# PKU-Alignment/SafeVLA

Measured on AMD Instinct MI355X. Metric: env-steps/sec through PPO-Lagrangian update, higher is better.
Workload: dtype bf16

## Files before the change

include/svla.h:

```cpp
#ifndef SVLA_H
#define SVLA_H
#include <stdint.h>
#ifdef __cplusplus
extern "C" {
#endif

typedef uint16_t svla_bf16;

typedef struct svla_dropout { unsigned seed, stream; float p; int row_mult; const unsigned* seed_dev; } svla_dropout;

int svla_gae_scan_f32(const float* rewards, const float* costs, const float* values, const float* c_values,
                      const float* masks, const float* next_v, const float* next_cv, double gamma, double tau, int T, int B,
                      float* ret, float* adv, float* c_ret, float* c_adv, void* stream);

int svla_ppo_lag_loss_fwd_bwd_f32(const float* logits, const float* values, const int64_t* actions, const float* old_logp,
                                  const float* adv, const float* c_adv, const float* returns, const float* old_values,
                                  int rows, int A, float lam, float clip, float value_coef, float action_w, float ent_coef,
                                  int use_clipped_value, float inv_n, float* dlogits, float* dvalues, double* sums,
                                  void* stream);
int svla_value_mse_fwd_bwd_f32(const float* values, const float* returns, const float* old_values, float clip, int rows, float coef,
                               float inv_n, float* dvalues, double* sums, void* stream);
int svla_hlgauss_fwd_bwd_f32(const float* logits, const float* target, const float* dvalue, int rows, int NB, float vmin, float vmax,
                             float sigma, float coef, float inv_n, float* values_out, float* dlogits, double* sums, void* stream);
int svla_ce_loss_fwd_bwd_f32(const float* logits, const long* target, int rows, int A, long ignore_index, const float* n_valid,
                             float* dlogits, double* sums, void* stream);

int svla_small_linear_fwd_f32(const float* x, const float* W, const float* bias, int rows, int N, int D, int T, int B,
                              float* out, void* stream);
int svla_small_linear_bwd_f32(const float* x, const float* W, const float* dout, int rows, int N, int D, int T, int B,
                              int accumulate_dx, float* dx, float* dW, float* db, void* stream);

int svla_norm_fwd_bf16(const svla_bf16* x, int xG, int xGS, int xOFF, const float* gamma, const float* beta, float eps, int rows,
                       int D, int rms, int relu, const float* tok, int tok_group, svla_bf16* y, int yG, int yGS, int yOFF,
                       float* mean, float* rstd, void* stream);
int svla_norm_bwd_bf16(const svla_bf16* dy, int dyG, int dyGS, int dyOFF, const svla_bf16* x, int xG, int xGS, int xOFF,
                       const float* gamma, const float* beta, const float* mean, const float* rstd, int rows, int D, int rms,
                       int relu, int tok_group, const svla_bf16* dres, svla_bf16* dx, int dxG, int dxGS, int dxOFF, float* dgamma,
                       float* dbeta, float* dtok, svla_bf16* dx_drop, const svla_dropout* drop, void* stream);

#define SVLA_RELU_BITS_BYTES(M, N) ((((long)(M) + 31) / 32) * 32 * ((long)(N) / 8))
int svla_gemm_nt_bf16(const svla_bf16* A, long lda, const svla_bf16* B, long ldb, const float* bias, const svla_bf16* residual,
                      long ldr, const svla_bf16* relu_mask, long ldm, void* C, long ldc, int M, int N, int K, int act,
                      int out_f32, float alpha, unsigned char* relu_bits_out, const unsigned char* relu_bits,
                      const svla_dropout* drop, void* stream);
int svla_gemm_force_small_tile(int on);
int svla_gemm_nt_rmsa_bf16(const svla_bf16* A, long lda, const svla_bf16* B, long ldb, const float* bias, const svla_bf16* residual, long ldr,
                           void* C, long ldc, int M, int N, int K, int act, float eps, const svla_dropout* drop, void* stream);
int svla_gemm_last_kernel(char* name, int cap, int* mnk);
int svla_asm_launch_raw(const char* name, const void* kernarg, int kernarg_bytes, int grid, int block, void* stream);
int svla_gemm_tn_f32acc(const svla_bf16* dY, long ldy, const svla_bf16* X, long ldx, float* dW, long ldw, float* db, int M, int N,
                        int K, void* stream);
int svla_colsum_bf16(const svla_bf16* dY, long ldy, int M, int N, int row_stride, float* db, void* stream);

int svla_gemm_f32(const float* A, long sam, long sak, const float* B, long sbn, long sbk, const float* bias, const float* residual,
                  long ldr, const float* mask, long ldm, float* C, long ldc, int M, int N, int K, int act, int accumulate, float alpha,
                  const svla_dropout* drop, void* stream);
int svla_colsum_f32(const float* X, long ldx, int M, int N, int row_stride, float* out, void* stream);

int svla_attn_fwd_bf16(const svla_bf16* Q, const svla_bf16* K, const svla_bf16* V, long ld, svla_bf16* O, long ldo, float* LSE,
                       int rows, int S, int H, int head_dim, float scale, int mask_mode, const int* traj, const float* bias,
                       const unsigned char* kvalid, int Sq, long ldq, int kv_rows, const svla_dropout* drop, void* stream);
int svla_attn_bwd_bf16(const svla_bf16* Q, const svla_bf16* K, const svla_bf16* V, long ld, const svla_bf16* O, long ldo,
                       const float* LSE, const svla_bf16* dO, long lddo, svla_bf16* dQ, svla_bf16* dK, svla_bf16* dV, long ldd,
                       int rows, int S, int H, int head_dim, float scale, int mask_mode, const int* traj, const float* bias,
                       const unsigned char* kvalid, int Sq, long ldq, long lddq, float* D_ws, const svla_dropout* drop,
                       void* stream);
int svla_attn_bwd_two_pass(int on);

int svla_replay_calls(int n, const int* fn_ids, const int* arg_offsets, const unsigned long long* args, int* failed_at);

int svla_acting_stage(const void* tok_src, void* tok_dst, long tok_bytes, const int64_t* pa_src, int64_t* pa_dst, const float* mask_src, float* mask_dst,
                      const int64_t* hand_src, int64_t* hand_dst, const int64_t* ts_src, int64_t* ts_dst, const int64_t* ids_src, int64_t* ids_dst, int64_t* am_dst,
                      unsigned char* am8_dst, unsigned char* kvalid_dst, int64_t* t_dev, int B, int L, int max_steps, int t, int* seed0, int* seed1, int* seed2,
                      int seed_inc, void* stream);

int svla_group_begin(int members);
int svla_group_member(int member);
int svla_group_end(void* stream);
int svla_group_stats(long* grouped, long* single);
int svla_replay_calls_grouped(int n, int members, const int* fn_ids, const int* arg_offsets, const unsigned long long* const* args, void* stream,
                              int* failed_at);
int svla_replay_abi_stamp(unsigned long long* stamp);

int svla_det_config(int slot, float* f32_base, long long* i64_shadow, long n);
int svla_det_finalize(float* f32, long long* i64_shadow, long n, void* stream);
int svla_det_bypass_count(unsigned long long* count, int reset);
int svla_det_set_grid(int frac_bits);

int svla_attn_fp8_quant(const svla_bf16* qkv, long ld, int rows, int S, int H, int head_dim, unsigned char* ws, float* scales,
                        void* stream);
int svla_attn_fp8_fwd(const unsigned char* ws, const float* scales, svla_bf16* O, long ldo, float* LSE, int rows, int S, int H,
                      int head_dim, float scale, const svla_dropout* drop, void* stream);
int svla_attn_fp8_bwd(const unsigned char* ws, const float* scales, const svla_bf16* O, long ldo, const float* LSE, const svla_bf16* dO,
                      long lddo, unsigned char* gws, float* gscale, float* D, svla_bf16* dQ, svla_bf16* dK, svla_bf16* dV, long ldd,
                      int rows, int S, int H, int head_dim, float scale, const svla_dropout* drop, void* stream);

int svla_feat_to_tokens(const float* feat, int R, int C, int P, int cam, int ncam, svla_bf16* out, void* stream);
int svla_fusion_fill(const float* fusion_token, const svla_bf16* text, const int* gid, int R, int S, int L, int text_off, int D,
                     svla_bf16* x0, void* stream);
int svla_fusion_text_bwd(const svla_bf16* dx0, const int* gid, int T, int B, int S, int L, int text_off, int D, float* dtext,
                         void* stream);
int svla_decoder_embed_fwd(const svla_bf16* xf, long xf_row_stride, const float* act_tab, const float* hand_tab,
                           const float* div_term, const int64_t* prev_actions, const float* masks, const int64_t* hand,
                           const int64_t* time_step, int T, int B, int n_actions, int D, svla_bf16* out, void* stream);
int svla_decoder_embed_bwd(const svla_bf16* dout, const int64_t* prev_actions, const float* masks, const int64_t* hand, int T,
                           int B, int n_actions, int D, svla_bf16* dxf, long dxf_row_stride, float* d_act_tab, float* d_hand_tab,
                           void* stream);
int svla_rows_add_bf16(svla_bf16* dst, long dst_ld, const svla_bf16* src, long src_ld, int rows, int D, void* stream);
int svla_zero_bytes(void* p, long bytes, void* stream);
int svla_kv_append_bf16(const svla_bf16* src, long ld_src, svla_bf16* cache, long cache_rows, int width, const int64_t* t_dev, int B,
                        void* stream);
int svla_swiglu_fwd(const svla_bf16* ab, long M, int Hd, svla_bf16* g, void* stream);
int svla_swiglu_bwd(const svla_bf16* ab, const svla_bf16* dg, long M, int Hd, svla_bf16* dab, void* stream);
int svla_row_hash_u8(const unsigned char* rows, long n_rows, int row_bytes, int64_t* out, void* stream);
int svla_embed_gather_f32_bf16(const float* table, const int64_t* ids, long n, int D, svla_bf16* out, void* stream);

int svla_normalize_u8_f32(const unsigned char* x, long n, const float* mean3, const float* std3, float* y, void* stream);
int svla_patchify_u8_bf16(const unsigned char* frames, int B, int H, int W, int crop_x, int P, int gh, int gw, int KP,
                          const float* mean3, const float* std3, svla_bf16* out, void* stream);
int svla_vit_tokens(const svla_bf16* patch, const float* cls, const float* pos, int B, int NP, int C, svla_bf16* y, void* stream);
// ... 75 lines not shown
```

safevla_amd/model.py:

```python
import math
import os
from typing import Dict, List, Optional, Tuple

import numpy as np

import torch
import torch.nn as nn

from . import ops
from .api import CategoricalDistr, SafeActorCriticOutput
from .losses import HLGaussLoss
from .text import GoalTokenizer, bytes_to_str

N_ACTIONS = 20
D = 512
DINO = 384
NPATCH = 84
TEXT_OFF = 1 + 2 * NPATCH
MAX_ACTING_WINDOW = 1024
TEXT_ENCODER_DIMS = {"t5-small": 512, "SigLIPBase": 768, "SigLIPLarge": 1024}
BF16, F32 = torch.bfloat16, torch.float32
import os as _os0
_NO_COMPRESSOR_BITS = _os0.environ.get("SVLA_NO_COMPRESSOR_BITS", "0") == "1"

# ... 57 lines not shown
    if init == "ones":
        return torch.ones(shape)
    if init == "zeros":
        return torch.zeros(shape)
    if init == "tok":
        return 0.1 * torch.rand(shape, generator=g)
    if init == "emb":
        return (torch.rand(shape, generator=g) * 2 - 1) * 0.01
    if init == "lin":
        fan_in = int(np.prod(shape[1:]))
        return (torch.rand(shape, generator=g) * 2 - 1) / math.sqrt(fan_in)
    if init == "actor":
        w = torch.empty(shape)
        nn.init.orthogonal_(w, gain=0.01)
        return w
    if init == "critic":
        w = torch.empty(shape)
        nn.init.orthogonal_(w)
        return w
    raise KeyError(init)


class Tower(nn.Module):

    def __init__(self, arena: _Arena, device, n_fusion_layers=3, n_decoder_layers=3, max_steps=500, critic_type="linear",
                 precision="bf16", dino_dim=DINO, text_encoder="t5-small", d_model=512, n_heads=8, n_heads_decoder=None):
        super().__init__()
        n_heads_decoder = n_heads if n_heads_decoder is None else n_heads_decoder
        if d_model % 64 or d_model > 1024 or d_model % n_heads or d_model % n_heads_decoder or max(d_model // n_heads, d_model // n_heads_decoder) > 128:
            raise NotImplementedError(f"transformer width {d_model} with {n_heads} / {n_heads_decoder} heads")
        D = self.D = d_model
        H = self.H = n_heads
        self.Hdec = n_heads_decoder
        self.hdim, self.hdim_dec = d_model // n_heads, d_model // n_heads_decoder
        HD = self.dec_hidden = 256 * ((int(2 * 4 * d_model / 3) + 255) // 256)
        self.dino_dim = dino_dim
        if text_encoder not in TEXT_ENCODER_DIMS:
            raise NotImplementedError("Only SigLIP and T5 text encoders are supported.")
        self.text_encoder_name, self.text_dim = text_encoder, TEXT_ENCODER_DIMS[text_encoder]
        if precision not in ("bf16", "fp32"):
            raise ValueError(f"precision must be 'bf16' (MFMA product path) or 'fp32' (verification mode), got {precision!r}")
        self.precision, self.adt = precision, (F32 if precision == "fp32" else BF16)
        if critic_type not in ("linear", "mlp", "discrete"):
            print(f"Unknown critic type: {critic_type}")
            raise NotImplementedError
        self.critic_type = critic_type
        self.arena = arena
        self.device_ = device
        if not 1 <= int(max_steps) <= MAX_ACTING_WINDOW:
            raise ValueError(f"max_steps = {max_steps}: the KV-cache window of the acting step is limited to {MAX_ACTING_WINDOW} steps")
        self.max_steps = max_steps
        self.time_step_counter = 0
        self.prune_last = True
        self.fp8_attention = False
        self.dropout_p = 0.1
        self.t5_dropout = True
        self.drop_seed_base = 0x5AFE + 977 * len(arena.specs)
        self._fwd_count = 0
        dec = arena.declare
        ve = self.visual_encoder = _NS()
        dec(ve, "fusion_token", (D,), "tok")
        dec(ve, "visual_sensor_token_raw_navigation_camera", (D,), "tok")
        dec(ve, "visual_sensor_token_raw_manipulation_camera", (D,), "tok")
        ve.text_adapter = _seq(3)
        dec(ve.text_adapter[0], "weight", (D, self.text_dim), "lin"); dec(ve.text_adapter[0], "bias", (D,), "zeros")
        dec(ve.text_adapter[1], "weight", (D,), "ones"); dec(ve.text_adapter[1], "bias", (D,), "zeros")
        ve.visual_compressor = _seq(4)
        dec(ve.visual_compressor[0], "weight", (D, dino_dim, 1, 1), "lin"); dec(ve.visual_compressor[0], "bias", (D,), "zeros")
        dec(ve.visual_compressor[2], "weight", (D, D, 1, 1), "lin"); dec(ve.visual_compressor[2], "bias", (D,), "zeros")
        ve.visual_adapter = _seq(3)
        dec(ve.visual_adapter[0], "weight", (D, D), "lin"); dec(ve.visual_adapter[0], "bias", (D,), "zeros")
        dec(ve.visual_adapter[1], "weight", (D,), "ones"); dec(ve.visual_adapter[1], "bias", (D,), "zeros")
        ve.fusion_xformer = _NS()
        ve.fusion_xformer.layers = nn.ModuleList()
        for _ in range(n_fusion_layers):
            l = _NS()
            l.self_attn = _NS()
            dec(l.self_attn, "in_proj_weight", (3 * D, D), "lin"); dec(l.self_attn, "in_proj_bias", (3 * D,), "zeros")
            l.self_attn.out_proj = _NS()
            dec(l.self_attn.out_proj, "weight", (D, D), "lin"); dec(l.self_attn.out_proj, "bias", (D,), "zeros")
            l.linear1 = _NS(); dec(l.linear1, "weight", (2048, D), "lin"); dec(l.linear1, "bias", (2048,), "zeros")
            l.linear2 = _NS(); dec(l.linear2, "weight", (D, 2048), "lin"); dec(l.linear2, "bias", (D,), "zeros")
            l.norm1 = _NS(); dec(l.norm1, "weight", (D,), "ones"); dec(l.norm1, "bias", (D,), "zeros")
            l.norm2 = _NS(); dec(l.norm2, "weight", (D,), "ones"); dec(l.norm2, "bias", (D,), "zeros")
            ve.fusion_xformer.layers.append(l)
        if text_encoder == "t5-small":
            ve.text_encoder = T5Frozen(device)
        else:
            from .siglip_text import SIGLIP_TEXT_PRESETS, SigLIPTextFrozen
            ve.text_encoder = SigLIPTextFrozen(device, **SIGLIP_TEXT_PRESETS[text_encoder])
        self.object_in_hand_embed = _NS(); dec(self.object_in_hand_embed, "weight", (3, D), "emb")
        self.last_actions_embed = _NS(); dec(self.last_actions_embed, "weight", (N_ACTIONS + 2, D), "emb")
        self.time_encoder = _NS()
        self.time_encoder.register_buffer("div_term", torch.exp(torch.arange(0, D, 2) * (-math.log(10000.0) / D)).to(device))
        self.decoder = _NS()
        self.decoder.layers = nn.ModuleList()
        for _ in range(n_decoder_layers):
            l = _NS()
            l.attention = _NS()
            for n in ("wq", "wk", "wv"):
                setattr(l.attention, n, _NS()); dec(getattr(l.attention, n), "weight", (D, D), "lin")
            l.attention.wo = _NS(); dec(l.attention.wo, "weight", (D, D), "lin")
            l.feed_forward = _NS()
            l.feed_forward.w1 = _NS(); l.feed_forward.w2 = _NS(); l.feed_forward.w3 = _NS()
            dec(l.feed_forward.w1, "weight", (HD, D), "lin")
            dec(l.feed_forward.w3, "weight", (HD, D), "lin")
# ... 90 lines not shown

    def _ensure_caches(self, B: int):
        D, H, HD = self.D, self.H, self.dec_hidden
        if getattr(self, "_kv", None) is None or self._kv[0].shape[0] < B:
            self._kv_version = getattr(self, "_kv_version", 0) + 1
            self._kv = [torch.zeros(B, self.max_steps, 2 * D, device=self.device_, dtype=self.adt) for _ in self.decoder.layers]

    def cache_select(self, keep: list):
        if getattr(self, "_kv", None) is not None:
            idx = torch.as_tensor(keep, device=self.device_, dtype=torch.long)
            self._kv = [c[idx].contiguous() for c in self._kv]
            self._kv_version = getattr(self, "_kv_version", 0) + 1

    def run_forward(self, prep: "Prep", need_grad: bool):
        D, H, HD = self.D, self.H, self.dec_hidden
        SCF, SCD = self.hdim ** -0.5, self.hdim_dec ** -0.5
        T, B, R, S, L, U = prep.T, prep.B, prep.R, prep.S, prep.L, prep.U
        if T > 1 or need_grad or not getattr(prep, "acting", True) or self.time_step_counter >= self.max_steps:
            self.time_step_counter = 0
        ve, w = self.visual_encoder, self._w
        M2, M = R * 2 * NPATCH, R * S
        c = {}
        c["drop_seed"], site = self._drop_sites()
        tok = prep.tokens.view(M2, self.dino_dim)
        bits = need_grad and self.adt == BF16 and not _NO_COMPRESSOR_BITS
        c1b = torch.empty(ops.relu_bits_bytes(M2, D), device=self.device_, dtype=torch.uint8) if bits else None
        c2b = torch.empty(ops.relu_bits_bytes(M2, D), device=self.device_, dtype=torch.uint8) if bits else None
        c1 = ops.gemm_nt(tok, w["c1"], M2, D, self.dino_dim, bias=ve.visual_compressor[0].bias, act=ops.ACT_RELU, relu_bits_out=c1b)
        c2 = ops.gemm_nt(c1, w["c2"], M2, D, D, bias=ve.visual_compressor[2].bias, act=ops.ACT_RELU, relu_bits_out=c2b)
        a1 = ops.gemm_nt(c2, w["va"], M2, D, D, bias=ve.visual_adapter[0].bias)
        x = torch.empty(R, S, D, device=self.device_, dtype=self.adt)
        _, va_mean, va_rstd = ops.norm_fwd(a1, ve.visual_adapter[1].weight, ve.visual_adapter[1].bias, 1e-5, M2, relu=True,
                                           tok=self._camtok, tok_group=NPATCH, y=x, ymap=(2 * NPATCH, S, 1), D=D)
        t5_seed = c["drop_seed"] if self.t5_dropout else None
        key = getattr(prep, "ids_key", None)
        if t5_seed is None and key is not None and getattr(self, "_t5_cache", (None, None))[0] == key:
            t5 = self._t5_cache[1]
        else:
            t5 = ve.text_encoder.encode(prep.ids, getattr(prep, "attn_mask_u8", None) if getattr(prep, "attn_mask_u8", None) is not None else prep.attn_mask,
                                        drop_seed=t5_seed, drop_p=self.dropout_p, dtype=self.adt,
                                        seed_dev=getattr(self, "_seed_dev", None), fused=getattr(self, "t5_fused", None))
            self._t5_cache = (key, t5) if (t5_seed is None and key is not None) else (None, None)
        ta = ops.gemm_nt(t5, w["ta"], U * L, D, self.text_dim, bias=ve.text_adapter[0].bias)
        tf, ta_mean, ta_rstd = ops.norm_fwd(ta, ve.text_adapter[1].weight, ve.text_adapter[1].bias, 1e-5, U * L, relu=True, D=D)
        ops.fusion_fill(ve.fusion_token, tf, prep.gid, x, R, S, L, TEXT_OFF)
        c.update(c1=c1, c2=c2, c1b=c1b, c2b=c2b, a1=a1, va=(va_mean, va_rstd), t5=t5, ta=ta, ta_stats=(ta_mean, ta_rstd))
        xf = x.view(M, D)
        fl = []
        nfl = len(ve.fusion_xformer.layers)
        xf_stride = S * D
        for i, l in enumerate(ve.fusion_xformer.layers):
            if i == nfl - 1 and self.prune_last:
                b_in = l.self_attn.in_proj_bias
                kv = ops.gemm_nt(xf, w[f"f{i}.in"][D:], M, 2 * D, D, bias=b_in[D:])
                q0 = ops.gemm_nt(xf, w[f"f{i}.in"][:D], R, D, D, bias=b_in[:D], lda=S * D)
                ao, lse = ops.attn_fwd(q0, kv, kv[:, D:], 2 * D, R, S, H, SCF, save_lse=need_grad, Sq=1, ldq=D, drop=site(i, 0), head_dim=self.hdim)
                h1 = ops.gemm_nt(ao, w[f"f{i}.out"], R, D, D, bias=l.self_attn.out_proj.bias, residual=xf, ldr=S * D, drop=site(i, 1, S))
                x1, m1, r1 = ops.norm_fwd(h1, l.norm1.weight, l.norm1.bias, 1e-5, R, save_stats=need_grad, D=D)
                f1 = ops.gemm_nt(x1, w[f"f{i}.l1"], R, 2048, D, bias=l.linear1.bias, act=ops.ACT_RELU, drop=site(i, 2, S))
                h2 = ops.gemm_nt(f1, w[f"f{i}.l2"], R, D, 2048, bias=l.linear2.bias, residual=x1, drop=site(i, 3, S))
                xo, m2, r2 = ops.norm_fwd(h2, l.norm2.weight, l.norm2.bias, 1e-5, R, save_stats=need_grad, D=D)
                if need_grad:
                    fl.append(dict(pruned=True, x=xf, kv=kv, q0=q0, ao=ao, lse=lse, h1=h1, x1=x1, n1=(m1, r1), f1=f1, h2=h2, n2=(m2, r2)))
                xf, xf_stride = xo, D
                continue
            qkv = ops.gemm_nt(xf, w[f"f{i}.in"], M, 3 * D, D, bias=l.self_attn.in_proj_bias)
            f8 = None
            if self.fp8_attention and self.adt == BF16 and S <= 256 and self.hdim == 64:
                f8 = ops.attn_fp8_quant(qkv, 3 * D, R, S, H)
                ao, lse = ops.attn_fp8_fwd(f8, SCF, save_lse=need_grad, drop=site(i, 0))
                qkv = None
            else:
                ao, lse = ops.attn_fwd(qkv, qkv[:, D:], qkv[:, 2 * D:], 3 * D, R, S, H, SCF, save_lse=need_grad, drop=site(i, 0), head_dim=self.hdim)
            h1 = ops.gemm_nt(ao, w[f"f{i}.out"], M, D, D, bias=l.self_attn.out_proj.bias, residual=xf, drop=site(i, 1))
            x1, m1, r1 = ops.norm_fwd(h1, l.norm1.weight, l.norm1.bias, 1e-5, M, save_stats=need_grad, D=D)
            f1b = torch.empty(ops.relu_bits_bytes(M, 2048), device=x1.device, dtype=torch.uint8) if (need_grad and self.adt == BF16) else None
            f1 = ops.gemm_nt(x1, w[f"f{i}.l1"], M, 2048, D, bias=l.linear1.bias, act=ops.ACT_RELU, relu_bits_out=f1b, drop=site(i, 2))
            h2 = ops.gemm_nt(f1, w[f"f{i}.l2"], M, D, 2048, bias=l.linear2.bias, residual=x1, drop=site(i, 3))
            xo, m2, r2 = ops.norm_fwd(h2, l.norm2.weight, l.norm2.bias, 1e-5, M, save_stats=need_grad, D=D)
            if need_grad:
                fl.append(dict(pruned=False, x=xf, qkv=qkv, f8=f8, ao=ao, lse=lse, h1=h1, x1=x1, n1=(m1, r1), f1=f1, f1b=f1b, h2=h2, n2=(m2, r2)))
            xf = xo
        c["fusion"] = fl
        j = torch.empty(R, D, device=self.device_, dtype=self.adt)
        ops.decoder_embed_fwd(xf, xf_stride, self.last_actions_embed.weight, self.object_in_hand_embed.weight,
                              self.time_encoder.div_term, prep.prev_actions, prep.masks, prep.hand, prep.time_step, T, B, j)
        xd = j
        dl = []
        if T == 1 and not need_grad and getattr(prep, "acting", True):
            if self.hdim_dec != 64:
                raise NotImplementedError("KV-cached single steps need 64-wide decoder heads (MFMA / decode attention kernels)")
            t = self.time_step_counter
            self._ensure_caches(B)
            t_dev = getattr(self, "_t_dev", None)
            if t_dev is None:
                start = torch.clamp(t - prep.time_step, min=0)
                kvalid = (torch.arange(t + 1, device=self.device_)[None, :] >= start[:, None]).to(torch.uint8).contiguous()
                S_att = t + 1
            else:
                kvalid = getattr(prep, "kvalid_static", None)
                if kvalid is None:
                    ar = self._ar_steps
                    kvalid = ((ar[None, :] <= t_dev) & (ar[None, :] >= torch.clamp(t_dev - prep.time_step, min=0)[:, None])).to(torch.uint8).contiguous()
                S_att = self.max_steps
            fused = self.adt == BF16 and getattr(self, "rms_fused", True)
            if fused:
                self.refresh_folded()
            for i, l in enumerate(self.decoder.layers):
                if fused:
                    qkv = ops.gemm_nt_rmsa(xd, self._wg[f"d{i}.qkv"], B, 3 * D, D, 1e-5)
                else:
                    n1, _, _ = ops.norm_fwd(xd, l.attention_norm.weight, None, 1e-5, B, rms=True, save_stats=False, D=D)
                    qkv = ops.gemm_nt(n1, w[f"d{i}.qkv"], B, 3 * D, D)
                cache = self._kv[i]
                if t_dev is None:
                    cache[:B, t].copy_(qkv[:, D:])
# ... 104 lines not shown
        ops.gemm_tn_acc(dy, c["nf"], dw["dout"], R, D, D)
        dnf = ops.gemm_nt(dy, wt["dout"], R, D, D)
        dx = ops.norm_bwd(dnf, c["xd_last"], self.decoder.norm.weight, None, None, c["rf"], R, g(self.decoder.norm.weight), None, rms=True, D=D)
        for i in reversed(range(len(self.decoder.layers))):
            l, a = self.decoder.layers[i], c["dec"][i]
            ops.gemm_tn_acc(dx, a["g"], dw[f"d{i}.w2"], R, D, HD)
            dg = ops.gemm_nt(dx, wt[f"d{i}.w2"], R, HD, D)
            dab = ops.swiglu_bwd(a["ab"], dg, R, HD)
            ops.gemm_tn_acc(dab, a["n2"], dw[f"d{i}.w13"], R, 2 * HD, D)
            dn2 = ops.gemm_nt(dab, wt[f"d{i}.w13"], R, D, 2 * HD)
            dh = ops.norm_bwd(dn2, a["h"], l.ffn_norm.weight, None, None, a["r2"], R, g(l.ffn_norm.weight), None, rms=True, dres=dx, D=D)
            ops.gemm_tn_acc(dh, a["ao"], dw[f"d{i}.wo"], R, D, D)
            dao = ops.gemm_nt(dh, wt[f"d{i}.wo"], R, D, D)
            dqkv = torch.empty(R, 3 * D, device=dev, dtype=self.adt)
            q = a["qkv"]
            ops.attn_bwd(q, q[:, D:], q[:, 2 * D:], 3 * D, a["ao"], D, a["lse"], dao, D, dqkv, dqkv[:, D:], dqkv[:, 2 * D:], 3 * D,
                         B, T, self.Hdec, SCD, mask_mode=ops.MASK_BLOCK_CAUSAL, traj=prep.traj_bt, head_dim=self.hdim_dec)
            ops.gemm_tn_acc(dqkv, a["n1"], dw[f"d{i}.qkv"], R, 3 * D, D)
            dn1 = ops.gemm_nt(dqkv, wt[f"d{i}.qkv"], R, D, 3 * D)
            dx = ops.norm_bwd(dn1, a["x"], l.attention_norm.weight, None, None, a["r1"], R, g(l.attention_norm.weight), None, rms=True, dres=dh, D=D)
        pruned = bool(c["fusion"]) and c["fusion"][-1]["pruned"]
        if pruned:
            dxf = torch.empty(R, D, device=dev, dtype=self.adt)
            ops.decoder_embed_bwd(dx, prep.prev_actions, prep.masks, prep.hand, T, B, dxf, D, g(self.last_actions_embed.weight),
                                  g(self.object_in_hand_embed.weight))
            dyf = dxf
        else:
            dxf = ops.zeros(R, S, D, device=dev, dtype=self.adt)
            ops.decoder_embed_bwd(dx, prep.prev_actions, prep.masks, prep.hand, T, B, dxf, S * D, g(self.last_actions_embed.weight),
                                  g(self.object_in_hand_embed.weight))
            dyf = dxf.view(M, D)
        site = self._site_fn(c.get("drop_seed"))
        drop_scale = 1.0 / (1.0 - self.dropout_p) if c.get("drop_seed") is not None else 1.0
        def masked_like(t, on):
            return torch.empty_like(t) if on else None
        for i in reversed(range(len(ve.fusion_xformer.layers))):
            l, a = ve.fusion_xformer.layers[i], c["fusion"][i]
            if a["pruned"]:
                d3, d1 = site(i, 3, S), site(i, 1, S)
                df = masked_like(a["h2"], d3 is not None)
                dh2 = ops.norm_bwd(dyf, a["h2"], l.norm2.weight, l.norm2.bias, a["n2"][0], a["n2"][1], R, g(l.norm2.weight), g(l.norm2.bias),
                                   dx_drop=df, drop=d3, D=D)
                df = dh2 if df is None else df
                ops.gemm_tn_acc(df, a["f1"], dw[f"f{i}.l2"], R, D, 2048, db=g(l.linear2.bias))
                df1 = ops.gemm_nt(df, wt[f"f{i}.l2"], R, 2048, D, relu_mask=a["f1"], alpha=drop_scale)
                ops.gemm_tn_acc(df1, a["x1"], dw[f"f{i}.l1"], R, 2048, D, db=g(l.linear1.bias))
                dx1 = ops.gemm_nt(df1, wt[f"f{i}.l1"], R, D, 2048, residual=dh2)
                da = masked_like(a["h1"], d1 is not None)
                dh1 = ops.norm_bwd(dx1, a["h1"], l.norm1.weight, l.norm1.bias, a["n1"][0], a["n1"][1], R, g(l.norm1.weight), g(l.norm1.bias),
                                   dx_drop=da, drop=d1, D=D)
                da = dh1 if da is None else da
                ops.gemm_tn_acc(da, a["ao"], dw[f"f{i}.out"], R, D, D, db=g(l.self_attn.out_proj.bias))
                dao = ops.gemm_nt(da, wt[f"f{i}.out"], R, D, D)
                dq0 = torch.empty(R, D, device=dev, dtype=self.adt)
                dkv = torch.empty(M, 2 * D, device=dev, dtype=self.adt)
                kv = a["kv"]
                ops.attn_bwd(a["q0"], kv, kv[:, D:], 2 * D, a["ao"], D, a["lse"], dao, D, dq0, dkv, dkv[:, D:], 2 * D, R, S, H, SCF, head_dim=self.hdim,
                             Sq=1, ldq=D, lddq=D, drop=site(i, 0))
                gb = g(l.self_attn.in_proj_bias)
                ops.gemm_tn_acc(dkv, a["x"], dw[f"f{i}.in"][D:], M, 2 * D, D, db=gb[D:])
                ops.gemm_tn_acc(dq0, a["x"], dw[f"f{i}.in"][:D], R, D, D, ldx=S * D, db=gb[:D])
                dyf = ops.gemm_nt(dkv, wt[f"f{i}.in"][:, D:], M, D, 2 * D)
                t0 = ops.gemm_nt(dq0, wt[f"f{i}.in"][:, :D], R, D, D, residual=dh1)
                ops.rows_add(dyf, S * D, t0, D, R, D)
                c["fusion"][i] = None
                continue
            d3, d1 = site(i, 3), site(i, 1)
            df = masked_like(a["h2"], d3 is not None)
            dh2 = ops.norm_bwd(dyf, a["h2"], l.norm2.weight, l.norm2.bias, a["n2"][0], a["n2"][1], M, g(l.norm2.weight), g(l.norm2.bias),
                               dx_drop=df, drop=d3, D=D)
            df = dh2 if df is None else df
            ops.gemm_tn_acc(df, a["f1"], dw[f"f{i}.l2"], M, D, 2048, db=g(l.linear2.bias))
            if a["f1b"] is not None:
                df1 = ops.gemm_nt(df, wt[f"f{i}.l2"], M, 2048, D, relu_bits=a["f1b"], alpha=drop_scale)
            else:
                df1 = ops.gemm_nt(df, wt[f"f{i}.l2"], M, 2048, D, relu_mask=a["f1"], alpha=drop_scale)
            ops.gemm_tn_acc(df1, a["x1"], dw[f"f{i}.l1"], M, 2048, D, db=g(l.linear1.bias))
            dx1 = ops.gemm_nt(df1, wt[f"f{i}.l1"], M, D, 2048, residual=dh2)
            del df1, df
            da = masked_like(a["h1"], d1 is not None)
            dh1 = ops.norm_bwd(dx1, a["h1"], l.norm1.weight, l.norm1.bias, a["n1"][0], a["n1"][1], M, g(l.norm1.weight), g(l.norm1.bias),
                               dx_drop=da, drop=d1, D=D)
            da = dh1 if da is None else da
            ops.gemm_tn_acc(da, a["ao"], dw[f"f{i}.out"], M, D, D, db=g(l.self_attn.out_proj.bias))
            dao = ops.gemm_nt(da, wt[f"f{i}.out"], M, D, D)
            dqkv = torch.empty(M, 3 * D, device=dev, dtype=self.adt)
            q = a["qkv"]
            if a.get("f8") is not None:
                ops.attn_fp8_bwd(a["f8"], a["ao"], a["lse"], dao, dqkv, dqkv[:, D:], dqkv[:, 2 * D:], 3 * D, SCF, drop=site(i, 0))
            else:
                ops.attn_bwd(q, q[:, D:], q[:, 2 * D:], 3 * D, a["ao"], D, a["lse"], dao, D, dqkv, dqkv[:, D:], dqkv[:, 2 * D:], 3 * D,
                             R, S, H, SCF, drop=site(i, 0), head_dim=self.hdim)
            ops.gemm_tn_acc(dqkv, a["x"], dw[f"f{i}.in"], M, 3 * D, D, db=g(l.self_attn.in_proj_bias))
            dyf = ops.gemm_nt(dqkv, wt[f"f{i}.in"], M, D, 3 * D, residual=dh1)
            c["fusion"][i] = None
        dx0 = dyf
        ops.colsum_acc(dx0, g(ve.fusion_token), R, D, row_stride=S)
        dtf = ops.zeros(U * L, D, device=dev, dtype=F32)
        if ops.det_active():
            dtf_sh = torch.zeros(U * L * D, device=dev, dtype=torch.int64)
            ops.det_config(1, dtf, dtf_sh)
            try:
                ops.fusion_text_bwd(dx0, prep.gid, T, B, S, L, TEXT_OFF, dtf)
                ops.det_finalize(dtf, dtf_sh)
            finally:
                ops.det_config(1, None, None)
        else:
            ops.fusion_text_bwd(dx0, prep.gid, T, B, S, L, TEXT_OFF, dtf)
        dtf_b = torch.empty(U * L, D, device=dev, dtype=self.adt)
        ops.cast_bf16(dtf, dtf_b)
        dta = ops.norm_bwd(dtf_b, c["ta"], ve.text_adapter[1].weight, ve.text_adapter[1].bias, c["ta_stats"][0], c["ta_stats"][1], U * L,
                           g(ve.text_adapter[1].weight), g(ve.text_adapter[1].bias), relu=True, D=D)
        ops.gemm_tn_acc(dta, c["t5"], dw["ta"], U * L, D, self.text_dim, db=g(ve.text_adapter[0].bias))
        da1 = ops.norm_bwd(dx0, c["a1"], ve.visual_adapter[1].weight, ve.visual_adapter[1].bias, c["va"][0], c["va"][1], M2,
                           g(ve.visual_adapter[1].weight), g(ve.visual_adapter[1].bias), relu=True, dtok=self._dcamtok,
# ... 489 lines not shown
```

safevla_amd/ops.py:

```python
import ctypes
import os
import struct
from typing import Optional, Tuple

import torch

from ._lib import lib

BF16 = torch.bfloat16
F32 = torch.float32

MASK_NONE, MASK_BLOCK_CAUSAL = 0, 1
ACT_NONE, ACT_RELU, ACT_GELU = 0, 1, 2


class LaunchPlan:

    def __init__(self):
        self.calls, self.keep = [], []

    def __enter__(self):
        global _REC
        assert _REC is None and lib().recorder is None, "launch recording is not re-entrant"
        _REC = self
# ... 350 lines not shown
        return colsum_f32(dY, db, M, N, row_stride=row_stride, ldx=ldy if ldy is not None else dY.stride(-2))
    lib().call("svla_colsum_bf16", _p(dY), ldy if ldy is not None else dY.stride(-2), M, N, row_stride, _p(db), _stream())


def _f32_cols(t, W):
    return t[:, :W].float().contiguous()


def _attn96_on_mfma(S, bias) -> bool:
    return S <= 256 and bias is None and os.environ.get("SVLA_ATTN96_F32", "0") != "1"


def attn_fwd(q, k, v, ld, rows, S, H, scale, out=None, ldo=None, mask_mode=MASK_NONE, traj=None, bias=None, kvalid=None,
             save_lse=True, Sq=0, ldq=0, kv_rows=0, drop=None, head_dim=64):
    nq = Sq if Sq > 0 else S
    W = H * head_dim
    if head_dim != 64 and q.dtype != F32 and not (head_dim == 96 and _attn96_on_mfma(S, bias)):
        q32, k32, v32 = _f32_cols(q, W), _f32_cols(k, W), _f32_cols(v, W)
        o32, lse = attn_fwd(q32, k32, v32, W, rows, S, H, scale, mask_mode=mask_mode, traj=traj, bias=bias, kvalid=kvalid, save_lse=save_lse, Sq=Sq,
                            ldq=W if Sq > 0 else 0, kv_rows=kv_rows, drop=drop, head_dim=head_dim)
        if out is None:
            return o32.to(q.dtype), lse
        out[:, :W].copy_(o32)
        return out, lse
    if out is None:
        out = torch.empty(rows * nq, W, device=q.device, dtype=q.dtype)
    ldo = ldo if ldo is not None else out.stride(-2)
    lse = torch.empty(rows, H, nq, device=q.device, dtype=F32) if save_lse else None
    lib().call("svla_attn_fwd_f32" if q.dtype == F32 else "svla_attn_fwd_bf16", _p(q), _p(k), _p(v), ld, _p(out), ldo, _p(lse), rows, S, H, int(head_dim), float(scale), mask_mode,
               _p(traj), _p(bias), _p(kvalid), int(Sq), int(ldq), int(kv_rows), _d(drop), _stream())
    return out, lse


def attn_bwd(q, k, v, ld, o, ldo, lse, do, lddo, dq, dk, dv, ldd, rows, S, H, scale, mask_mode=MASK_NONE, traj=None,
             bias=None, kvalid=None, Sq=0, ldq=0, lddq=0, d_ws=None, drop=None, head_dim=64):
    if head_dim != 64 and q.dtype != F32 and not (head_dim == 96 and _attn96_on_mfma(S, bias)):
        W = H * head_dim
        q32, k32, v32, o32, do32 = (_f32_cols(t, W) for t in (q, k, v, o, do))
        dq32, dk32, dv32 = torch.empty_like(q32), torch.empty_like(k32), torch.empty_like(v32)
        attn_bwd(q32, k32, v32, W, o32, W, lse, do32, W, dq32, dk32, dv32, W, rows, S, H, scale, mask_mode=mask_mode, traj=traj, kvalid=kvalid, Sq=Sq,
                 ldq=W if Sq > 0 else 0, lddq=W if Sq > 0 else 0, drop=drop, head_dim=head_dim)
        dq[:, :W].copy_(dq32); dk[:, :W].copy_(dk32); dv[:, :W].copy_(dv32)
        return
    if q.dtype == F32:
        lib().call("svla_attn_bwd_f32", _p(q), _p(k), _p(v), ld, _p(o), ldo, _p(lse), _p(do), lddo, _p(dq), _p(dk), _p(dv), ldd, rows, S, H, int(head_dim),
                   float(scale), mask_mode, _p(traj), _p(kvalid), int(Sq), int(ldq), int(lddq), _d(drop), _stream())
        return
    if d_ws is None:
        d_ws = torch.empty(rows * H * (Sq or S), device=q.device, dtype=F32)
    lib().call("svla_attn_bwd_bf16", _p(q), _p(k), _p(v), ld, _p(o), ldo, _p(lse), _p(do), lddo, _p(dq), _p(dk), _p(dv), ldd,
               rows, S, H, int(head_dim), float(scale), mask_mode, _p(traj), _p(bias), _p(kvalid), int(Sq), int(ldq), int(lddq), _p(d_ws), _d(drop), _stream())


_DET_SLOTS = [None, None]


def det_config(slot: int, f32: Optional[torch.Tensor], shadow: Optional[torch.Tensor]) -> None:
    if f32 is None:
        lib().call("svla_det_config", int(slot), None, None, 0)
        _DET_SLOTS[slot] = None
        return
    assert f32.dtype == F32 and shadow.dtype == torch.int64 and shadow.numel() == f32.numel() and f32.is_contiguous()
    lib().call("svla_det_config", int(slot), f32.data_ptr(), shadow.data_ptr(), f32.numel())
    _DET_SLOTS[slot] = (f32, shadow)


def det_active() -> bool:
    return _DET_SLOTS[0] is not None


def det_finalize(f32: torch.Tensor, shadow: torch.Tensor) -> None:
    lib().call("svla_det_finalize", _p(f32), _p(shadow), f32.numel(), _stream())


def det_set_grid(frac_bits: int) -> None:
    lib().call("svla_det_set_grid", int(frac_bits))


def det_grid_bits(n_total: int) -> int:
    import math
    return max(36, min(52, 52 - max(0, math.ceil(math.log2(16384.0 / max(1, int(n_total)))))))


def det_bypass_count(reset: bool = True) -> int:
    c = ctypes.c_ulonglong(0)
    lib().call("svla_det_bypass_count", ctypes.byref(c), int(bool(reset)))
    return int(c.value)


def _fp8_sp(S: int) -> int:
    return 64 if S <= 64 else 128 if S <= 128 else 192 if S <= 192 else 256


class Fp8QKV:
    __slots__ = ("ws", "scales", "rows", "S", "H")

    def __init__(self, ws, scales, rows, S, H):
        self.ws, self.scales, self.rows, self.S, self.H = ws, scales, rows, S, H


def attn_fp8_quant(qkv, ld, rows, S, H) -> Fp8QKV:
    _chk(qkv, BF16, "qkv")
    ws = torch.empty(rows * H * 6 * _fp8_sp(S) * 64, device=qkv.device, dtype=torch.uint8)
    scales = torch.empty(rows * H * 3, device=qkv.device, dtype=F32)
    lib().call("svla_attn_fp8_quant", _p(qkv), ld, rows, S, H, 64, _p(ws), _p(scales), _stream())
    return Fp8QKV(ws, scales, rows, S, H)
# ... 311 lines not shown
```

Baseline: 7763.

## Absorb K/V projections into query for pruned last fusion layer attention

```diff
diff --git a/include/svla.h b/include/svla.h
--- a/include/svla.h
+++ b/include/svla.h
@@ -66,6 +66,12 @@
                        const unsigned char* kvalid, int Sq, long ldq, long lddq, float* D_ws, const svla_dropout* drop,
                        void* stream);
 int svla_attn_bwd_two_pass(int on);
+int svla_attn_q1_fwd_bf16(const svla_bf16* X, long ldx, const svla_bf16* QT, svla_bf16* C, float* SIG, float* P, int R, int S, float scale,
+                          const svla_dropout* drop, void* stream);
+int svla_attn_q1_bwd_bf16(const svla_bf16* X, long ldx, const svla_bf16* QT, const svla_bf16* DC, const float* DSIG, const float* P,
+                          svla_bf16* DX, long lddx, svla_bf16* DQT, int R, int S, float scale, const svla_dropout* drop, void* stream);
+int svla_head_expand_bf16(const svla_bf16* v, long ldv, int R, svla_bf16* E, const float* bias, float* dot, const float* sigma, svla_bf16* vs, void* stream);
+int svla_head_pick_bf16(const svla_bf16* G, int R, const float* sigma, const float* bias, svla_bf16* out, long ldo, void* stream);
 
 int svla_replay_calls(int n, const int* fn_ids, const int* arg_offsets, const unsigned long long* args, int* failed_at);
 
diff --git a/safevla_amd/csrc/attn_q1.hip b/safevla_amd/csrc/attn_q1.hip
--- /dev/null
+++ b/safevla_amd/csrc/attn_q1.hip
@@ -0,0 +1,303 @@
+#include "attn_common.h"
+
+#define Q1_D 512
+#define Q1_H 8
+#define Q1_WAVES 8
+#define Q1_THREADS (Q1_WAVES * 64)
+#define Q1_SMAX 256
+#define Q1_SLOTS (Q1_SMAX / Q1_WAVES)
+#define Q1_RED_FLOATS (Q1_H * Q1_D)
+#define Q1_LDS_FWD ((size_t)(Q1_SMAX * Q1_H + 4 * Q1_RED_FLOATS) * sizeof(float))
+#define Q1_LDS_BWD ((size_t)(2 * Q1_SMAX * Q1_H + 4 * Q1_RED_FLOATS) * sizeof(float))
+
+__device__ __forceinline__ void q1_unpack(bf16x8 v, float (&f)[8]) {
+    const u32x4 w = __builtin_bit_cast(u32x4, v);
+#pragma unroll
+    for (int i = 0; i < 4; ++i) { f[2 * i] = bf_lo(w[i]); f[2 * i + 1] = bf_hi(w[i]); }
+}
+
+__device__ __forceinline__ void q1_token_head_products(const bf16_t* __restrict__ X, const bf16_t* __restrict__ V, int S, float mul, float* out, int w, int lane) {
+    constexpr int NT = Q1_SMAX / (16 * Q1_WAVES), NK = Q1_D / 32;
+    const int ql = lane & 15, g = lane >> 4;
+    const bf16_t* vb = V + (size_t)(ql & (Q1_H - 1)) * Q1_D + 8 * g;
+    bf16x8 a[NT][NK], b[NK];
+#pragma unroll
+    for (int tt = 0; tt < NT; ++tt) {
+        const bf16_t* xa = X + (size_t)min((w + Q1_WAVES * tt) * 16 + ql, S - 1) * Q1_D + 8 * g;
+#pragma unroll
+        for (int kk = 0; kk < NK; ++kk) a[tt][kk] = *(const bf16x8*)(xa + kk * 32);
+    }
+#pragma unroll
+    for (int kk = 0; kk < NK; ++kk) b[kk] = *(const bf16x8*)(vb + kk * 32);
+#pragma unroll
+    for (int tt = 0; tt < NT; ++tt) {
+        const int j0 = (w + Q1_WAVES * tt) * 16;
+        f32x4 acc = {0.f, 0.f, 0.f, 0.f};
+#pragma unroll
+        for (int kk = 0; kk < NK; ++kk) acc = mfma16(a[tt][kk], b[kk], acc);
+        if (ql < Q1_H) {
+#pragma unroll
+            for (int i = 0; i < 4; ++i) {
+                const int j = j0 + 4 * g + i;
+                if (j < S) out[j * Q1_H + ql] = acc[i] * mul;
+            }
+        }
+    }
+}
+
+__device__ __forceinline__ void q1_load_slices(const bf16_t* __restrict__ X, int S, int w, int lane, bf16x8 (&xr)[Q1_SLOTS]) {
+#pragma unroll
+    for (int t = 0; t < Q1_SLOTS; ++t) {
+        const int j = min(w + Q1_WAVES * t, S - 1);
+        xr[t] = *(const bf16x8*)(X + (size_t)j * Q1_D + lane * 8);
+    }
+}
+
+__device__ __forceinline__ void q1_token_sums(const bf16x8 (&xr)[Q1_SLOTS], const float* coef, int S, int w, float (&acc)[Q1_H][8]) {
+#pragma unroll
+    for (int h = 0; h < Q1_H; ++h)
+#pragma unroll
+        for (int e = 0; e < 8; ++e) acc[h][e] = 0.f;
+#pragma unroll
+    for (int t = 0; t < Q1_SLOTS; ++t) {
+        const int j = w + Q1_WAVES * t;
+        if (j < S) {
+            const f32x4 c0 = *(const f32x4*)(coef + j * Q1_H), c1 = *(const f32x4*)(coef + j * Q1_H + 4);
+            float x[8];
+            q1_unpack(xr[t], x);
+#pragma unroll
+            for (int h = 0; h < 4; ++h)
+#pragma unroll
+                for (int e = 0; e < 8; ++e) { acc[h][e] += c0[h] * x[e]; acc[h + 4][e] += c1[h] * x[e]; }
+        }
+    }
+}
+
+__device__ __forceinline__ void q1_red_store(const float (&acc)[Q1_H][8], float* buf, int lane) {
+#pragma unroll
+    for (int h = 0; h < Q1_H; ++h) {
+        *(f32x4*)(buf + h * Q1_D + lane * 8) = f32x4{acc[h][0], acc[h][1], acc[h][2], acc[h][3]};
+        *(f32x4*)(buf + h * Q1_D + lane * 8 + 4) = f32x4{acc[h][4], acc[h][5], acc[h][6], acc[h][7]};
+    }
+}
+__device__ __forceinline__ void q1_red_add(float (&acc)[Q1_H][8], const float* buf, int lane) {
+#pragma unroll
+    for (int h = 0; h < Q1_H; ++h) {
+        const f32x4 a = *(const f32x4*)(buf + h * Q1_D + lane * 8), b = *(const f32x4*)(buf + h * Q1_D + lane * 8 + 4);
+#pragma unroll
+        for (int e = 0; e < 4; ++e) { acc[h][e] += a[e]; acc[h][e + 4] += b[e]; }
+    }
+}
+__device__ __forceinline__ void q1_reduce_write(float (&acc)[Q1_H][8], float* red, int w, int lane, bf16_t* __restrict__ out) {
+    if (w >= 4) q1_red_store(acc, red + (w - 4) * Q1_RED_FLOATS, lane);
+    __syncthreads();
+    if (w < 4) q1_red_add(acc, red + w * Q1_RED_FLOATS, lane);
+    if (w == 2 || w == 3) q1_red_store(acc, red + w * Q1_RED_FLOATS, lane);
+    __syncthreads();
+    if (w < 2) q1_red_add(acc, red + (w + 2) * Q1_RED_FLOATS, lane);
+    if (w == 1) q1_red_store(acc, red + Q1_RED_FLOATS, lane);
+    __syncthreads();
+    if (w == 0) {
+        q1_red_add(acc, red + Q1_RED_FLOATS, lane);
+#pragma unroll
+        for (int h = 0; h < Q1_H; ++h) *(bf16x8*)(out + h * Q1_D + lane * 8) = pack8(acc[h]);
+    }
+}
+
+struct Q1Args {
+    const bf16_t* X; long ldx;
+    const bf16_t* QT;
+    bf16_t* C; float* SIG; float* P;
+    const bf16_t* DC; const float* DSIG;
+    bf16_t* DX; long lddx; bf16_t* DQT;
+    int S; float scale; DropCfg drop;
+};
+
+__global__ void __launch_bounds__(Q1_THREADS, 1) attn_q1_fwd_kernel(Q1Args p) {
+    extern __shared__ __attribute__((aligned(16))) char smem[];
+    float* sc = (float*)smem;
+    float* red = sc + Q1_SMAX * Q1_H;
+    const int w = __builtin_amdgcn_readfirstlane(threadIdx.x >> 6), lane = threadIdx.x & 63, S = p.S;
+    const size_t r = blockIdx.x;
+    const DropCfg drop = drop_resolve(p.drop);
+    const bf16_t* X = p.X + r * p.ldx;
+    q1_token_head_products(X, p.QT + r * (Q1_H * Q1_D), S, p.scale, sc, w, lane);
+    bf16x8 xr[Q1_SLOTS];
+    q1_load_slices(X, S, w, lane, xr);
+    __syncthreads();
+    {
+        const int h = w;
+        float v[Q1_SMAX / 64], m = -INFINITY, sum = 0.f, sig = 0.f;
+#pragma unroll
+        for (int i = 0; i < Q1_SMAX / 64; ++i) {
+            const int j = lane + 64 * i;
+            v[i] = j < S ? sc[j * Q1_H + h] : -INFINITY;
+            m = fmaxf(m, v[i]);
+        }
+        m = wave_max(m);
+#pragma unroll
+        for (int i = 0; i < Q1_SMAX / 64; ++i) { v[i] = __expf(v[i] - m); sum += v[i]; }
+        const float inv = 1.f / wave_sum(sum);
+        const unsigned long long e0 = att_drop_row(S, Q1_H, (int)r, h, 0);
+#pragma unroll
+        for (int i = 0; i < Q1_SMAX / 64; ++i) {
+            const int j = lane + 64 * i;
+            if (j < S) {
+                const float pr = v[i] * inv;
+                const float pd = (!drop.thr || att_keep1(drop, e0 + j)) ? pr * drop.scale : 0.f;
+                p.P[(r * Q1_H + h) * S + j] = pr;
+                sc[j * Q1_H + h] = pd;
+                sig += pd;
+            }
+        }
+        sig = wave_sum(sig);
+        if (lane == 0) p.SIG[r * Q1_H + h] = sig;
+    }
+    __syncthreads();
+    float acc[Q1_H][8];
+    q1_token_sums(xr, sc, S, w, acc);
+    q1_reduce_write(acc, red, w, lane, p.C + r * (Q1_H * Q1_D));
+}
+
+__global__ void __launch_bounds__(Q1_THREADS, 1) attn_q1_bwd_kernel(Q1Args p) {
+    extern __shared__ __attribute__((aligned(16))) char smem[];
+    float* dsb = (float*)smem;
+    float* pdb = dsb + Q1_SMAX * Q1_H;
+    float* red = pdb + Q1_SMAX * Q1_H;
+    const int w = __builtin_amdgcn_readfirstlane(threadIdx.x >> 6), lane = threadIdx.x & 63, S = p.S;
+    const size_t r = blockIdx.x;
+    const DropCfg drop = drop_resolve(p.drop);
+    const bf16_t* X = p.X + r * p.ldx;
+    q1_token_head_products(X, p.DC + r * (Q1_H * Q1_D), S, 1.f, dsb, w, lane);
+    bf16x8 xr[Q1_SLOTS];
+    q1_load_slices(X, S, w, lane, xr);
+    __syncthreads();
+    {
+        const int h = w;
+        const float dsig = p.DSIG[r * Q1_H + h];
+        const unsigned long long e0 = att_drop_row(S, Q1_H, (int)r, h, 0);
+        float pr[Q1_SMAX / 64], dp[Q1_SMAX / 64], delta = 0.f;
+#pragma unroll
+        for (int i = 0; i < Q1_SMAX / 64; ++i) {
+            const int j = lane + 64 * i;
+            pr[i] = 0.f; dp[i] = 0.f;
+            if (j < S) {
+                pr[i] = p.P[(r * Q1_H + h) * S + j];
+                const bool keep = !drop.thr || att_keep1(drop, e0 + j);
+                dp[i] = keep ? (dsb[j * Q1_H + h] + dsig) * drop.scale : 0.f;
+                pdb[j * Q1_H + h] = keep ? pr[i] * drop.scale : 0.f;
+                delta += pr[i] * dp[i];
+            }
+        }
+        delta = wave_sum(delta);
+#pragma unroll
+        for (int i = 0; i < Q1_SMAX / 64; ++i) {
+            const int j = lane + 64 * i;
+            if (j < S) dsb[j * Q1_H + h] = p.scale * pr[i] * (dp[i] - delta);
+        }
+    }
+    __syncthreads();
+    {
+        float acc[Q1_H][8];
+        q1_token_sums(xr, dsb, S, w, acc);
+        q1_reduce_write(acc, red, w, lane, p.DQT + r * (Q1_H * Q1_D));
+    }
+    float qf[Q1_H][8], cf[Q1_H][8];
+    const bf16_t* QT = p.QT + r * (Q1_H * Q1_D) + lane * 8;
+    const bf16_t* DC = p.DC + r * (Q1_H * Q1_D) + lane * 8;
+#pragma unroll
+    for (int h = 0; h < Q1_H; ++h) {
+        q1_unpack(*(const bf16x8*)(QT + h * Q1_D), qf[h]);
+        q1_unpack(*(const bf16x8*)(DC + h * Q1_D), cf[h]);
+    }
+    bf16_t* DX = p.DX + r * p.lddx;
+#pragma unroll 1
+    for (int j = w; j < S; j += Q1_WAVES) {
+        const f32x4 s0 = *(const f32x4*)(dsb + j * Q1_H), s1 = *(const f32x4*)(dsb + j * Q1_H + 4);
+        const f32x4 d0 = *(const f32x4*)(pdb + j * Q1_H), d1 = *(const f32x4*)(pdb + j * Q1_H + 4);
+        float o[8];
+#pragma unroll
+        for (int e = 0; e < 8; ++e) o[e] = 0.f;
+#pragma unroll
+        for (int h = 0; h < 4; ++h)
+#pragma unroll
+            for (int e = 0; e < 8; ++e) {
+                o[e] += s0[h] * qf[h][e] + d0[h] * cf[h][e];
+                o[e] += s1[h] * qf[h + 4][e] + d1[h] * cf[h + 4][e];
+            }
+        *(bf16x8*)(DX + (size_t)j * Q1_D + lane * 8) = pack8(o);
+    }
+}
+
+static bool q1_shape_ok(int R, int S, long ldx) { return R > 0 && S > 0 && S <= Q1_SMAX && ldx >= (long)S * Q1_D && ldx % 8 == 0; }
+
+extern "C" int svla_attn_q1_fwd_bf16(const bf16_t* X, long ldx, const bf16_t* QT, bf16_t* C, float* SIG, float* P, int R, int S, float scale,
+                                     const svla_dropout* drop, void* stream) {
+    if (!X || !QT || !C || !SIG || !P || !q1_shape_ok(R, S, ldx)) return SVLA_EINVAL;
+    Q1Args p{};
+    p.X = X; p.ldx = ldx; p.QT = QT; p.C = C; p.SIG = SIG; p.P = P; p.S = S; p.scale = scale; p.drop = drop_cfg(drop);
+    return svla_launch<attn_q1_fwd_kernel>(dim3(R), dim3(Q1_THREADS), Q1_LDS_FWD, (hipStream_t)stream, p);
+}
+
+extern "C" int svla_attn_q1_bwd_bf16(const bf16_t* X, long ldx, const bf16_t* QT, const bf16_t* DC, const float* DSIG, const float* P,
+                                     bf16_t* DX, long lddx, bf16_t* DQT, int R, int S, float scale, const svla_dropout* drop, void* stream) {
+    if (!X || !QT || !DC || !DSIG || !P || !DX || !DQT || !q1_shape_ok(R, S, ldx) || !q1_shape_ok(R, S, lddx)) return SVLA_EINVAL;
+    Q1Args p{};
+    p.X = X; p.ldx = ldx; p.QT = QT; p.DC = DC; p.DSIG = DSIG; p.P = (float*)P; p.DX = DX; p.lddx = lddx; p.DQT = DQT;
+    p.S = S; p.scale = scale; p.drop = drop_cfg(drop);
+    return svla_launch<attn_q1_bwd_kernel>(dim3(R), dim3(Q1_THREADS), Q1_LDS_BWD, (hipStream_t)stream, p);
+}
+
+__global__ void __launch_bounds__(256) head_expand_kernel(const bf16_t* __restrict__ v, long ldv, int R, bf16_t* __restrict__ E, const float* __restrict__ bias,
+                                                          float* __restrict__ dot, const float* __restrict__ sigma, bf16_t* __restrict__ vs) {
+    const size_t r = (size_t)blockIdx.x * 4 + (threadIdx.x >> 6);
+    const int lane = threadIdx.x & 63, hl = lane >> 3;
+    if (r >= (size_t)R) return;
+    const bf16x8 x = *(const bf16x8*)(v + r * ldv + lane * 8);
+    const bf16x8 z = {0, 0, 0, 0, 0, 0, 0, 0};
+#pragma unroll
+    for (int h = 0; h < Q1_H; ++h) *(bf16x8*)(E + (r * Q1_H + h) * Q1_D + lane * 8) = h == hl ? x : z;
+    if (!bias && !sigma) return;
+    float f[8];
+    q1_unpack(x, f);
+    if (bias) {
+        float s = 0.f;
+#pragma unroll
+        for (int e = 0; e < 8; ++e) s += f[e] * bias[lane * 8 + e];
+        s += __shfl_xor(s, 1, 64); s += __shfl_xor(s, 2, 64); s += __shfl_xor(s, 4, 64);
+        if ((lane & 7) == 0) dot[r * Q1_H + hl] = s;
+    }
+    if (sigma) {
+        const float sg = sigma[r * Q1_H + hl];
+#pragma unroll
+        for (int e = 0; e < 8; ++e) f[e] *= sg;
+        *(bf16x8*)(vs + r * Q1_D + lane * 8) = pack8(f);
+    }
+}
+__global__ void __launch_bounds__(256) head_pick_kernel(const bf16_t* __restrict__ G, int R, const float* __restrict__ sigma, const float* __restrict__ bias,
+                                                        bf16_t* __restrict__ out, long ldo) {
+    const size_t r = (size_t)blockIdx.x * 4 + (threadIdx.x >> 6);
+    const int lane = threadIdx.x & 63, hl = lane >> 3;
+    if (r >= (size_t)R) return;
+    bf16x8 x = *(const bf16x8*)(G + (r * Q1_H + hl) * Q1_D + lane * 8);
+    if (sigma) {
+        float f[8];
+        q1_unpack(x, f);
+        const float sg = sigma[r * Q1_H + hl];
+#pragma unroll
+        for (int e = 0; e < 8; ++e) f[e] += sg * bias[lane * 8 + e];
+        x = pack8(f);
+    }
+    *(bf16x8*)(out + r * ldo + lane * 8) = x;
+}
+
+extern "C" int svla_head_expand_bf16(const bf16_t* v, long ldv, int R, bf16_t* E, const float* bias, float* dot, const float* sigma, bf16_t* vs, void* stream) {
+    if (!v || !E || R <= 0 || ldv < Q1_D || ldv % 8 || (bias && !dot) || (sigma && !vs)) return SVLA_EINVAL;
+    hipLaunchKernelGGL(head_expand_kernel, dim3((R + 3) / 4), dim3(256), 0, (hipStream_t)stream, v, ldv, R, E, bias, dot, sigma, vs);
+    return svla_launch_status();
+}
+extern "C" int svla_head_pick_bf16(const bf16_t* G, int R, const float* sigma, const float* bias, bf16_t* out, long ldo, void* stream) {
+    if (!G || !out || R <= 0 || ldo < Q1_D || ldo % 8 || (sigma && !bias)) return SVLA_EINVAL;
+    hipLaunchKernelGGL(head_pick_kernel, dim3((R + 3) / 4), dim3(256), 0, (hipStream_t)stream, G, R, sigma, bias, out, ldo);
+    return svla_launch_status();
+}
diff --git a/safevla_amd/model.py b/safevla_amd/model.py
--- a/safevla_amd/model.py
+++ b/safevla_amd/model.py
@@ -133,6 +133,7 @@
         self.max_steps = max_steps
         self.time_step_counter = 0
         self.prune_last = True
+        self.absorb_last = _os0.environ.get("SVLA_LAST_LAYER_KV", "0") != "1"
         self.fp8_attention = False
         self.dropout_p = 0.1
         self.t5_dropout = True
@@ -329,16 +330,25 @@
         for i, l in enumerate(ve.fusion_xformer.layers):
             if i == nfl - 1 and self.prune_last:
                 b_in = l.self_attn.in_proj_bias
-                kv = ops.gemm_nt(xf, w[f"f{i}.in"][D:], M, 2 * D, D, bias=b_in[D:])
                 q0 = ops.gemm_nt(xf, w[f"f{i}.in"][:D], R, D, D, bias=b_in[:D], lda=S * D)
-                ao, lse = ops.attn_fwd(q0, kv, kv[:, D:], 2 * D, R, S, H, SCF, save_lse=need_grad, Sq=1, ldq=D, drop=site(i, 0), head_dim=self.hdim)
+                absorbed = need_grad and self.absorb_last and self.adt == BF16 and self.hdim == 64 and H == 8 and S <= 256
+                if absorbed:
+                    eq, _, _ = ops.head_expand(q0, R)
+                    qt = ops.gemm_nt(eq, self._wt[f"f{i}.in"][:, D:2 * D], 8 * R, D, D)
+                    cc, sig, prob = ops.attn_q1_fwd(xf, S * D, qt, R, S, SCF, drop=site(i, 0))
+                    ao = ops.head_pick(ops.gemm_nt(cc, w[f"f{i}.in"][2 * D:], 8 * R, D, D), R, sigma=sig, bias=b_in[2 * D:])
+                    att = dict(absorbed=True, eq=eq, qt=qt, cc=cc, sig=sig, prob=prob)
+                else:
+                    kv = ops.gemm_nt(xf, w[f"f{i}.in"][D:], M, 2 * D, D, bias=b_in[D:])
+                    ao, lse = ops.attn_fwd(q0, kv, kv[:, D:], 2 * D, R, S, H, SCF, save_lse=need_grad, Sq=1, ldq=D, drop=site(i, 0), head_dim=self.hdim)
+                    att = dict(absorbed=False, kv=kv, lse=lse)
                 h1 = ops.gemm_nt(ao, w[f"f{i}.out"], R, D, D, bias=l.self_attn.out_proj.bias, residual=xf, ldr=S * D, drop=site(i, 1, S))
                 x1, m1, r1 = ops.norm_fwd(h1, l.norm1.weight, l.norm1.bias, 1e-5, R, save_stats=need_grad, D=D)
                 f1 = ops.gemm_nt(x1, w[f"f{i}.l1"], R, 2048, D, bias=l.linear1.bias, act=ops.ACT_RELU, drop=site(i, 2, S))
                 h2 = ops.gemm_nt(f1, w[f"f{i}.l2"], R, D, 2048, bias=l.linear2.bias, residual=x1, drop=site(i, 3, S))
                 xo, m2, r2 = ops.norm_fwd(h2, l.norm2.weight, l.norm2.bias, 1e-5, R, save_stats=need_grad, D=D)
                 if need_grad:
-                    fl.append(dict(pruned=True, x=xf, kv=kv, q0=q0, ao=ao, lse=lse, h1=h1, x1=x1, n1=(m1, r1), f1=f1, h2=h2, n2=(m2, r2)))
+                    fl.append(dict(pruned=True, x=xf, q0=q0, ao=ao, **att, h1=h1, x1=x1, n1=(m1, r1), f1=f1, h2=h2, n2=(m2, r2)))
                 xf, xf_stride = xo, D
                 continue
             qkv = ops.gemm_nt(xf, w[f"f{i}.in"], M, 3 * D, D, bias=l.self_attn.in_proj_bias)
@@ -549,15 +559,27 @@
                 da = dh1 if da is None else da
                 ops.gemm_tn_acc(da, a["ao"], dw[f"f{i}.out"], R, D, D, db=g(l.self_attn.out_proj.bias))
                 dao = ops.gemm_nt(da, wt[f"f{i}.out"], R, D, D)
-                dq0 = torch.empty(R, D, device=dev, dtype=self.adt)
-                dkv = torch.empty(M, 2 * D, device=dev, dtype=self.adt)
-                kv = a["kv"]
-                ops.attn_bwd(a["q0"], kv, kv[:, D:], 2 * D, a["ao"], D, a["lse"], dao, D, dq0, dkv, dkv[:, D:], 2 * D, R, S, H, SCF, head_dim=self.hdim,
-                             Sq=1, ldq=D, lddq=D, drop=site(i, 0))
                 gb = g(l.self_attn.in_proj_bias)
-                ops.gemm_tn_acc(dkv, a["x"], dw[f"f{i}.in"][D:], M, 2 * D, D, db=gb[D:])
-                ops.gemm_tn_acc(dq0, a["x"], dw[f"f{i}.in"][:D], R, D, D, ldx=S * D, db=gb[:D])
-                dyf = ops.gemm_nt(dkv, wt[f"f{i}.in"][:, D:], M, D, 2 * D)
+                if a["absorbed"]:
+                    w_in, wt_in, dw_in = w[f"f{i}.in"], wt[f"f{i}.in"], dw[f"f{i}.in"]
+                    edao, dsig, sdao = ops.head_expand(dao, R, bias=l.self_attn.in_proj_bias[2 * D:], sigma=a["sig"])
+                    dcc = ops.gemm_nt(edao, wt_in[:, 2 * D:], 8 * R, D, D)
+                    ops.gemm_tn_acc(edao, a["cc"], dw_in[2 * D:], 8 * R, D, D)
+                    ops.colsum_acc(sdao, gb[2 * D:], R, D)
+                    dyf, dqt = ops.attn_q1_bwd(a["x"], S * D, a["qt"], dcc, dsig, a["prob"], R, S, SCF, drop=site(i, 0))
+                    dyf = dyf.view(M, D)
+                    ops.gemm_tn_acc(a["eq"], dqt, dw_in[D:2 * D], 8 * R, D, D)
+                    dq0 = ops.head_pick(ops.gemm_nt(dqt, w_in[D:2 * D], 8 * R, D, D), R)
+                    ops.gemm_tn_acc(dq0, a["x"], dw_in[:D], R, D, D, ldx=S * D, db=gb[:D])
+                else:
+                    dq0 = torch.empty(R, D, device=dev, dtype=self.adt)
+                    dkv = torch.empty(M, 2 * D, device=dev, dtype=self.adt)
+                    kv = a["kv"]
+                    ops.attn_bwd(a["q0"], kv, kv[:, D:], 2 * D, a["ao"], D, a["lse"], dao, D, dq0, dkv, dkv[:, D:], 2 * D, R, S, H, SCF, head_dim=self.hdim,
+                                 Sq=1, ldq=D, lddq=D, drop=site(i, 0))
+                    ops.gemm_tn_acc(dkv, a["x"], dw[f"f{i}.in"][D:], M, 2 * D, D, db=gb[D:])
+                    ops.gemm_tn_acc(dq0, a["x"], dw[f"f{i}.in"][:D], R, D, D, ldx=S * D, db=gb[:D])
+                    dyf = ops.gemm_nt(dkv, wt[f"f{i}.in"][:, D:], M, D, 2 * D)
                 t0 = ops.gemm_nt(dq0, wt[f"f{i}.in"][:, :D], R, D, D, residual=dh1)
                 ops.rows_add(dyf, S * D, t0, D, R, D)
                 c["fusion"][i] = None
diff --git a/safevla_amd/ops.py b/safevla_amd/ops.py
--- a/safevla_amd/ops.py
+++ b/safevla_amd/ops.py
@@ -426,6 +426,42 @@
                rows, S, H, int(head_dim), float(scale), mask_mode, _p(traj), _p(bias), _p(kvalid), int(Sq), int(ldq), int(lddq), _p(d_ws), _d(drop), _stream())
 
 
+def attn_q1_fwd(x, ldx, qt, R, S, scale, drop=None):
+    _chk(x, BF16, "x")
+    _chk(qt, BF16, "qt")
+    c = torch.empty(8 * R, 512, device=x.device, dtype=BF16)
+    sig = torch.empty(R, 8, device=x.device, dtype=F32)
+    P = torch.empty(R, 8, S, device=x.device, dtype=F32)
+    lib().call("svla_attn_q1_fwd_bf16", _p(x), int(ldx), _p(qt), _p(c), _p(sig), _p(P), R, S, float(scale), _d(drop), _stream())
+    return c, sig, P
+
+
+def attn_q1_bwd(x, ldx, qt, dc, dsig, P, R, S, scale, drop=None):
+    for t, n in ((x, "x"), (qt, "qt"), (dc, "dc")):
+        _chk(t, BF16, n)
+    dx = torch.empty(R, S, 512, device=x.device, dtype=BF16)
+    dqt = torch.empty(8 * R, 512, device=x.device, dtype=BF16)
+    lib().call("svla_attn_q1_bwd_bf16", _p(x), int(ldx), _p(qt), _p(dc), _p(dsig), _p(P),
+               _p(dx), S * 512, _p(dqt), R, S, float(scale), _d(drop), _stream())
+    return dx, dqt
+
+
+def head_expand(v, R, bias=None, sigma=None, ldv=None):
+    _chk(v, BF16, "v")
+    E = torch.empty(8 * R, 512, device=v.device, dtype=BF16)
+    dot = torch.empty(R, 8, device=v.device, dtype=F32) if bias is not None else None
+    vs = torch.empty(R, 512, device=v.device, dtype=BF16) if sigma is not None else None
+    lib().call("svla_head_expand_bf16", _p(v), ldv if ldv is not None else v.stride(-2), R, _p(E), _p(bias), _p(dot), _p(sigma), _p(vs), _stream())
+    return E, dot, vs
+
+
+def head_pick(G, R, sigma=None, bias=None):
+    _chk(G, BF16, "G")
+    out = torch.empty(R, 512, device=G.device, dtype=BF16)
+    lib().call("svla_head_pick_bf16", _p(G), R, _p(sigma), _p(bias), _p(out), 512, _stream())
+    return out
+
+
 _DET_SLOTS = [None, None]
 
 
```

New measurement: 8139, median of 6. 4.8% higher.
